# spirlness/qt-raytracer

Hardware: AMD Instinct MI355X
Metric: Msamples/s (rays×bounces/s) at 1920×1080, 8 bounces; 1/2/4/8-GPU scaling (higher is better)
Workload: dtype f32

## Files before the change

### include/hippt.h

```cpp
#ifndef HIPPT_H
#define HIPPT_H

#include <stdbool.h>
#include <stdint.h>

#ifdef __cplusplus
extern "C" {
#endif

bool cudaPathTracerInit(int width, int height, const char **errorMessage);
bool cudaPathTracerRender(int frameIndex, int maxDepth, const unsigned int **hostPixels,
                          const char **errorMessage);
void cudaPathTracerShutdown(void);

bool hipPathTracerInit(int width, int height, const char **errorMessage);
bool hipPathTracerRender(int frameIndex, int maxDepth, const unsigned int **hostPixels,
                         const char **errorMessage);
void hipPathTracerShutdown(void);

typedef struct hipptCamera {
    float origin[3], llc[3], horizontal[3], vertical[3], u[3], v[3];
    float lens_radius;
    float reserved;
} hipptCamera;
// ... 113 lines not shown
    , HIPPT_OPT_LDS_TOP_NODES = 20
    , HIPPT_OPT_BVH_COLLAPSE = 21
    , HIPPT_OPT_BVH_NODE_COST = 22
    , HIPPT_OPT_BVH_LEAF4 = 23
    , HIPPT_OPT_RNG_TABLE = 24
    , HIPPT_OPT_PIXEL_FORMAT = 25
    , HIPPT_OPT_CAMERA_POOL = 26
    , HIPPT_OPT_FUSE_COMBINE = 27
    , HIPPT_OPT_ITEM_ORDER = 28
    , HIPPT_OPT_WAVEFRONT_SORT = 29
    , HIPPT_OPT_CHAIN = 30
    , HIPPT_OPT_CHAIN_AUDIT = 31
    , HIPPT_OPT_PIXEL_TILE = 32
    , HIPPT_OPT_QUERY_SLICE = 33
    , HIPPT_OPT_RENDER_PAD = 34
};
int hipptChainAudit(unsigned int *words, int maxWords);
enum { HIPPT_PIXEL_ARGB = 0, HIPPT_PIXEL_RGBA8 = 1 };
enum { HIPPT_INFO_LDS_TOP_BYTES = 100, HIPPT_INFO_BLOCKS_PER_CU = 101, HIPPT_INFO_CHUNK = 102,
       HIPPT_INFO_CHAIN_CAP = 103,
       HIPPT_INFO_UPDATE_DROPPED = 104 ,
       HIPPT_INFO_RENDER_PAD = 105 };
bool hipptSetOption(int key, long long value);
long long hipptGetOption(int key);
int hipptActiveBvhWidth(void);

const char *hipptLastError(void);

typedef struct hipptBvh hipptBvh;
hipptBvh *hipptBvhBuild(const float *verts, int numTris, float extentHint, const char **errorMessage);
int hipptBvhNodeCount(const hipptBvh *bvh);
int hipptBvhDepth(const hipptBvh *bvh);
void hipptBvhCopy(const hipptBvh *bvh, uint32_t *nodes, int *triOrder);
void hipptBvhFree(hipptBvh *bvh);
bool hipptBvhRefit(hipptBvh *bvh, const float *verts, int numTris, float extentHint, const char **errorMessage);
int hipptBvh4NodeCount(const hipptBvh *bvh);
int hipptBvh4Depth(const hipptBvh *bvh);
// ... 10 lines not shown
```

### qt-raytracer_amd/csrc/hippt_api.cpp

```cpp
#include "../../include/hippt.h"
#include "item_order.h"

#include <hip/hip_runtime.h>

#include <algorithm>
#include <atomic>
#include <cmath>
#include <condition_variable>
#include <cstdio>
#include <cstring>
#include <exception>
#include <memory>
#include <mutex>
#include <stdexcept>
#include <string>
#include <system_error>
#include <thread>
#include <utility>
#include <vector>

#include "bvh_builder.h"
#include "mesh_io.h"
#include "hippt_device.h"
#include "hippt_query.h"
#include "hippt_refit.h"
#include "hippt_slab.h"
#include "hippt_wavefront.h"

struct hipptBvh {
    hippt::Bvh bvh;
    hippt::Bvh4 bvh4;
    std::vector<uint32_t> bvh4q;
};

namespace {

using hippt::CameraF;

using hippt::kStatSlots;
using hippt::kStatWords;
// ... 210 lines not shown
    int leafExit = -1;
    int nodeExit = -1;
    int bvhWidth = 0;
    int stackCap = 0;
    int bvhQuant = -1;
    int ldsTopNodes = -1;
    bool rngTable = false;
    int pixelFormat = HIPPT_PIXEL_ARGB;
    int cameraPool = -1;
    int fuseCombine = -1;
    int itemOrder = -1;
    int pixelTile = -1;
    int chainBatches = -1;
    bool chainAudit = false;
    int renderPad = hippt::slab::kRenderPadDefault;
    long long querySlice = 0;
    std::vector<unsigned> auditWords;
    std::vector<std::pair<int, uint32_t *>> rngTables;
    struct SpareBuf {
        int device;
        void *ptr;
        size_t bytes;
    };
    std::vector<SpareBuf> spare;
    struct Update {
        float *stage[2] = {nullptr, nullptr};
        size_t floats = 0;
        int next = 0;
        std::vector<std::pair<int, hipEvent_t>> busy[2];
        bool hostStale = false;
        int staleBuf = 0;
        hipEvent_t staleEv = nullptr;
    } upd;
    unsigned activeTopBytes = 0;
    int activeBlocksPerCu = 0;
    int activeChunk = 0;
    int activeChainCap = 0;
    int activeRenderPad = 0;
    int activeWidth = 0;
    int blocksPerCu = 0;
    bool ldsScene = true;
    int pathMode = 0;
    unsigned wfSlots = 1u << 27;
    int wfSort = -1;
    hippt::BvhParams bvh;
    double traceMs = 0, combineMs = 0;
    int traceLaunches = 0, combineLaunches = 0;
};

State &S() {
    static State s;
    return s;
// ... 430 lines not shown
        !up(c.mats, s.scene.mats) || !up(c.nodes4, s.scene.nodes4) || !up(c.nodes4q, s.scene.nodes4q))
        return false;
    HIP_TRY(hipMalloc(&c.padDev, 16));
    HIP_TRY(hipMemcpy(c.padDev, &s.scene.pad, sizeof(float), hipMemcpyHostToDevice));
    c.sceneVersion = s.scene.version;
    return true;
}

constexpr float kRenderPadMinSine = 0.3f;
bool render_pad_holds(const SceneHost &sc, bool hostStale, const CameraF &cam) {
    const float M = hostStale ? sc.padSeed : std::max(sc.padSeed, sc.pad * 65536.0f);
    float o = 0.0f;
    for (int k = 0; k < 3; ++k) o = std::max(o, std::fabs(cam.origin[k]));
    const float reach = o + 1.5f * std::fabs(cam.lens_radius);
    return std::isfinite(reach) && reach <= M && sc.minEdgeSine >= kRenderPadMinSine;
}

unsigned packed_ref_bits(int numNodes, int numPrims) {
    const unsigned long long maxMag =
        std::max<unsigned long long>((unsigned long long)std::max(numNodes, 1) * 128ull,
                                     ((unsigned long long)numPrims << 4) + 16ull);
    unsigned bits = 1;
    while ((1ull << (bits - 1)) < maxMag) ++bits;
    return std::max(bits, 8u);
}

constexpr size_t kOrderTables = 4;

int cost_threads() { return int(std::max(1u, std::min(16u, std::thread::hardware_concurrency()))); }

// ... 529 lines not shown
    return true;
}

bool chain_same(const hippt::MeshParams &a, const hippt::MeshParams &b) {
    return a.nodes == b.nodes && a.tris == b.tris && a.shade == b.shade && a.mats == b.mats && a.stats == b.stats &&
           same_cam(a.cam, b.cam) && a.invW == b.invW && a.invH == b.invH && a.width == b.width &&
           a.height == b.height && a.y0 == b.y0 && a.bandRows == b.bandRows && a.rowStride == b.rowStride &&
           a.frames == b.frames && a.maxDepth == b.maxDepth && a.bandPixels == b.bandPixels &&
           a.totalItems == b.totalItems && a.stackDepth == b.stackDepth && a.numNodes == b.numNodes &&
           a.numTris == b.numTris && a.numMats == b.numMats && a.ldsScene == b.ldsScene && a.full == b.full &&
           a.waveThreshold == b.waveThreshold && a.chunk == b.chunk && a.leafExit == b.leafExit &&
           a.nodeExit == b.nodeExit && a.wide == b.wide && a.stackCap == b.stackCap && a.spillCap == b.spillCap &&
           a.spill == b.spill && a.topBytes == b.topBytes && a.refBits == b.refBits && a.runOrder == b.runOrder &&
           a.runCount == b.runCount && a.runTileShift == b.runTileShift && a.rngTable == b.rngTable && a.poolOffset == b.poolOffset &&
           a.poolWords == b.poolWords && a.comb.format == b.comb.format && a.padWord == b.padWord &&
           a.trimScale == b.trimScale;
}

bool launch_chained(Ctx &c, hippt::MeshParams &p, const char **err) {
    Ctx::Chain &ch = c.chain;
    p.chainEpoch = ch.epoch++;
    ch.lastOwn = p.chainSeq;
    ch.pendN = 0;
    if (!c.chainStartEv) HIP_TRY(hipEventCreateWithFlags(&c.chainStartEv, hipEventDisableTiming));
    if (!c.chainEndEv) HIP_TRY(hipEventCreateWithFlags(&c.chainEndEv, hipEventDisableTiming));
    EventPair ev;
    if (!next_events(c, ev, err)) return false;
    HIP_TRY(hipEventRecord(c.chainStartEv, c.stream));
    HIP_TRY(hipEventRecord(ev.a, c.stream));
    HIP_TRY(hippt::launch_mesh(p, int(ch.blocks), false, c.stream));
    HIP_TRY(hipEventRecord(ev.b, c.stream));
// ... 317 lines not shown
                        const bool lambertMega = s.pathMode == 0 && !s.scene.full;
                        p.leafExit = unsigned(s.leafExit >= 0 ? s.leafExit
                                              : ldsScene          ? (lambertMega ? 12 : 4)
                                              : fullMega          ? 12
                                              : lambertGlobal     ? 22
                                                                  : 17);
                        p.nodeExit = unsigned(s.nodeExit >= 0 ? s.nodeExit
                                              : ldsScene  ? 8
                                              : fullMega  ? 16
                                              : lambertGlobal ? 56
                                                              : 48);
                        p.wide = fmt;
                        p.stackCap = stackCap;
                        p.topBytes = topBytes;
                        p.refBits = ldsScene && wide ? packed_ref_bits(numNodes, numTris) : 0u;
                        const bool trims = s.pathMode == 0 && ldsScene && fmt == hippt::kWideFloat && s.renderPad != 0 &&
                                           render_pad_holds(s.scene, s.upd.hostStale, cam);
                        p.padWord = c.padDev;
                        p.trimScale = trims ? hippt::slab::trim_scale(s.renderPad) : 0.0f;
                        s.activeRenderPad = trims ? s.renderPad : 0;
                        p.rngTable = nullptr;
                        p.poolWords = poolWords;
                        if (s.pathMode == 0 && s.itemOrder != 0) {
                            const unsigned *table = nullptr;
                            const int tile = s.pixelTile >= 0 ? s.pixelTile : c.stride == 1 ? 8 : 0;
                            const unsigned tileShift = tile == 8 ? 3u : tile == 16 ? 4u : tile == 32 ? 5u : 6u;
                            if (!ensure_order(c, cam, nf, maxDepth, s.itemOrder == 1, tileShift, &table, err))
                                return false;
                            if (table) {
                                p.runOrder = table;
                                p.runCount = unsigned(c.runCosts.size());
                                p.runTileShift = c.orderKey.tileShift;
                            }
                        }
                        p.poolOffset = unsigned(hippt::mesh_lds_bytes(stackDepth, ldsScene ? numNodes : 0,
// ... 1197 lines not shown
        if (value != 0 && value != 1) return false;
        s.chainAudit = value == 1;
        return true;
    case HIPPT_OPT_PIXEL_TILE:
        if (value != -1 && value != 0 && value != 8 && value != 16 && value != 32) return false;
        s.pixelTile = int(value);
        return true;
    case HIPPT_OPT_QUERY_SLICE:
        if (value < 0 || value > (1LL << 28)) return false;
        s.querySlice = value;
        return true;
    case HIPPT_OPT_RENDER_PAD:
        if (value != 0 && (value < hippt::slab::kRenderPadMin || value > hippt::slab::kRenderPadMax)) return false;
        s.renderPad = int(value);
        return true;
    default: return false;
    }
} catch (const std::exception &e) {
    return false;
} catch (...) {
    return false;
}

extern "C" int hipptActiveBvhWidth(void) try {
    std::lock_guard<std::mutex> g(S().mu);
    return S().activeWidth;
} catch (const std::exception &e) {
    return 0;
} catch (...) {
    return 0;
// ... 24 lines not shown
    case HIPPT_OPT_LDS_TOP_NODES: return s.ldsTopNodes;
    case HIPPT_OPT_BVH_COLLAPSE: return s.bvh.collapse;
    case HIPPT_OPT_BVH_NODE_COST: return (long long)std::lround(s.bvh.nodeCost * 100.0f);
    case HIPPT_OPT_BVH_LEAF4: return s.bvh.maxLeaf4;
    case HIPPT_OPT_RNG_TABLE: return s.rngTable ? 1 : 0;
    case HIPPT_OPT_PIXEL_FORMAT: return s.pixelFormat;
    case HIPPT_OPT_CAMERA_POOL: return s.cameraPool;
    case HIPPT_OPT_FUSE_COMBINE: return s.fuseCombine;
    case HIPPT_OPT_ITEM_ORDER: return s.itemOrder;
    case HIPPT_OPT_WAVEFRONT_SORT: return s.wfSort;
    case HIPPT_OPT_CHAIN: return s.chainBatches;
    case HIPPT_OPT_CHAIN_AUDIT: return s.chainAudit ? 1 : 0;
    case HIPPT_OPT_PIXEL_TILE: return s.pixelTile;
    case HIPPT_OPT_QUERY_SLICE: return s.querySlice;
    case HIPPT_OPT_RENDER_PAD: return s.renderPad;
    case HIPPT_INFO_LDS_TOP_BYTES: return s.activeTopBytes;
    case HIPPT_INFO_BLOCKS_PER_CU: return s.activeBlocksPerCu;
    case HIPPT_INFO_CHUNK: return s.activeChunk;
    case HIPPT_INFO_CHAIN_CAP: return s.activeChainCap;
    case HIPPT_INFO_RENDER_PAD: return s.activeRenderPad;
    case HIPPT_INFO_UPDATE_DROPPED:
        for (Ctx &c : s.ctxs) {
            if (!c.rfUpdated) continue;
            unsigned w[2] = {0, 0};
            if (hipSetDevice(c.device) != hipSuccess || hipStreamSynchronize(c.stream) != hipSuccess ||
                hipMemcpy(w, c.rfWords, sizeof(w), hipMemcpyDeviceToHost) != hipSuccess) {
                (void)hipGetLastError();
                return -1;
            }
            return w[1];
        }
        return 0;
    default: return -1;
    }
} catch (const std::exception &e) {
// ... 107 lines not shown
```

### qt-raytracer_amd/csrc/hippt_device.h

```cpp
#pragma once

#include <hip/hip_runtime.h>

#include <cstdint>

namespace hippt {

struct CameraF {
    float origin[3], llc[3], horizontal[3], vertical[3], u[3], v[3];
    float lens_radius;
    float reserved;
};

struct Sphere4Params {
    float4 *accum;
    uint32_t *out;
    unsigned long long *stats;
    int width, height, y0, rows, rowStride;
    int firstFrame, frames, maxDepth;
    int format;
    uint32_t *hostOut;
};

enum { kPixelArgb = 0, kPixelRgba8 = 1 };

struct CombineParams {
    float4 *accum;
    uint32_t *out;
    const float *scratch;
    unsigned bandPixels, totalItems;
    int firstFrame, frames;
    int format;
};

struct HostFrame {
    uint32_t *host;
    int width, y0, stride;
};

struct MeshParams {
    const float4 *nodes;
    const float4 *tris;
    const float4 *shade;
    const float4 *mats;
    float *scratch;
    unsigned *queue;
    unsigned long long *stats;
    CameraF cam;
    float invW, invH;
    int width, height, y0, bandRows, rowStride;
    int firstFrame, frames, maxDepth;
    unsigned bandPixels, totalItems;
// ... 18 lines not shown
    const uint32_t *rngTable;
    unsigned poolOffset;
    int poolWords;
    CombineParams comb;
    unsigned *combCtr;
    unsigned *chainCtl;
    const unsigned long long *chainBox;
    unsigned chainSeq, chainEpoch, chainRun;
    unsigned chainSlots, chainShift, chainCap;
    int chainStep;
    unsigned chainPosted;
    unsigned chainGroup;
    unsigned *chainAudit;
    const float *padWord;
    float trimScale;
};

constexpr unsigned kChainSlotsMax = 32, kChainBlockWords = 8 * 32 + 32, kChainMarkerWord = 8 * 32;
constexpr unsigned kChainCtlWord = kChainSlotsMax * kChainBlockWords;
constexpr unsigned kChainBoxWord = kChainCtlWord + 128, kChainCtlWords = kChainBoxWord + 8 * 32;
constexpr unsigned kChainMaxShift = 27;
constexpr unsigned kWaveWords = 22;

struct ChainFlushParams {
    CombineParams comb;
    const float *scratch;
    const unsigned *ctl;
    unsigned epoch, lastSeq, slots, shift;
    int step;
    unsigned *audit;
// ... 39 lines not shown
```

### qt-raytracer_amd/csrc/hippt_kernels.hip

```cpp
#include "hippt_trace.h"

#include <algorithm>

#pragma clang fp contract(off)

namespace hippt {
namespace {
using namespace trace;

__device__ __forceinline__ unsigned q8(float c) {
    return unsigned(sqrtf(fminf(fmaxf(c, 0.0f), 1.0f)) * 255.0f);
}

__device__ __forceinline__ uint32_t pack_pixel(float r, float g, float b, int format) {
    if (format == kPixelRgba8) {
        const auto u8 = [](float c) { return unsigned(rintf(sqrtf(fminf(fmaxf(c, 0.0f), 1.0f)) * 255.0f)); };
        return (255u << 24) | (u8(b) << 16) | (u8(g) << 8) | u8(r);
    }
    return (255u << 24) | (q8(r) << 16) | (q8(g) << 8) | q8(b);
}

struct V3 {
    float x, y, z;
};
// ... 122 lines not shown
#endif

#ifndef HIPPT_NUM_SGPR
#define HIPPT_NUM_SGPR 96
#endif
#define HIPPT_SGPR_ATTR __attribute__((amdgpu_num_sgpr(HIPPT_NUM_SGPR)))

#ifndef HIPPT_REJECT_CAP
#define HIPPT_REJECT_CAP 0
#endif

#ifndef HIPPT_PACKED_KEYS
#define HIPPT_PACKED_KEYS 1
#endif

#ifndef HIPPT_LATE_CAM
#define HIPPT_LATE_CAM 0
#endif
#ifndef HIPPT_WIDE_WAVES_PER_EU
#define HIPPT_WIDE_WAVES_PER_EU 7
#endif
template <int UNROLL, bool HOST = false>
__device__ __forceinline__ void combine_pixel(const CombineParams &P, unsigned p, const HostFrame &H = HostFrame{}) {
    float4 acc = P.accum[p];
#pragma unroll UNROLL
    for (int fl = 0; fl < P.frames; ++fl) {
        const size_t k = size_t(fl) * P.bandPixels + p;
        const int f = P.firstFrame + fl;
        const float ff = float(f), fc = float(f + 1);
        const float3 L = *reinterpret_cast<const float3 *>(P.scratch + 3 * k);
// ... 185 lines not shown
    T.cur = kDone;
    T.sp = 0;
    T.leaf = 0;
    T.bestT = INFINITY;
    T.bestI = -1;
    T.bestO = 0x7fffffff;
    float tr = 1, tg = 1, tb = 1;
    bool need = true, fresh = false;
    constexpr unsigned CAP = FULL ? 0u : unsigned(HIPPT_REJECT_CAP);
    unsigned pend = 0;
    unsigned segs = 0, samples = 0;
    unsigned long long nvis = 0, ntest = 0;
    unsigned pc[kProfSlots] = {0};

    constexpr bool FINISH = POOL && !LDS_SCENE;
#ifdef HIPPT_DEBUG_RATE
    const unsigned long long rtStart = __builtin_amdgcn_s_memrealtime();
    unsigned rtBucket = 0, rtSegs0 = 0, rtSamples0 = 0;
    unsigned long long rtRounds = 0, rtLive = 0;
    auto rt_flush = [&](unsigned nb) {
        const unsigned long long a = wave_sum((unsigned long long)(samples - rtSamples0));
        const unsigned wsegs = CHAIN ? __builtin_amdgcn_readfirstlane(ww->segs) : 0u;
        const unsigned long long b = CHAIN ? (unsigned long long)(wsegs - rtSegs0) : wave_sum((unsigned long long)(segs - rtSegs0));
        rtSamples0 = samples;
        rtSegs0 = CHAIN ? wsegs : segs;
        if (__lane_id() == 0) {
            const unsigned k = ((blockIdx.x * 4u + (threadIdx.x >> 6)) % unsigned(kRateSlots) * unsigned(kRateBuckets) +
                                min(rtBucket, unsigned(kRateBuckets - 1))) * 5u;
            atomicAdd(&g_rate[k], a);
            atomicAdd(&g_rate[k + 1], b);
            atomicAdd(&g_rate[k + 2], rtRounds);
            atomicAdd(&g_rate[k + 3], rtLive);
            atomicAdd(&g_rate[k + 4], 1ull);
        }
        rtRounds = rtLive = 0;
        rtBucket = nb;
    };
#endif
    unsigned waveThr = unsigned(P.waveThreshold);
    bool combLeft = CHAIN ? int(__builtin_amdgcn_readfirstlane(cw->c1)) >= int(__builtin_amdgcn_readfirstlane(cw->c0))
                          : P.comb.bandPixels != 0;
    auto comb_step = [&]() { return CHAIN ? combine_chunk_chain(cw) : combine_chunk(P); };
    if (combLeft && (blockIdx.x & 1u) == 0 && threadIdx.x < 64u)
        while (combLeft) combLeft = comb_step();
    for (;;) {
        prof<STATS>(pc, 0);
#ifdef HIPPT_DEBUG_TIMELINE
        if (tlDrained) ++tlRounds;
#endif
#ifdef HIPPT_DEBUG_RATE
        {
            const unsigned nb = unsigned((__builtin_amdgcn_s_memrealtime() - rtStart) / 1000ull);
            if (nb != rtBucket) rt_flush(nb);
            ++rtRounds;
            rtLive += __popcll(__ballot(item != kNone));
        }
#endif
        if (POOL) {
            const unsigned long long m = __ballot(need);
            if (m) {
                const unsigned n = unsigned(__popcll(m));
                const unsigned rank = __builtin_amdgcn_mbcnt_hi(unsigned(m >> 32), __builtin_amdgcn_mbcnt_lo(unsigned(m), 0u));
                const unsigned avail = 64u - poolNext;
                const bool took = need;
                if (need && rank < avail) {
                    need = false;
                    pool_take<POOL>(P, pool, poolNext + rank, item, r, rng);
                }
                if (n > avail) {
                    unsigned it;
                    Ray c{};
                    uint32_t crng = 0;
                    if constexpr (CHAIN) {
                        WorkQueue Q = load_queue(&ww->Q);
                        unsigned raw = kNone, tItem = 0;
                        bool want = true;
                        for (;;) {
                            const unsigned t = __builtin_amdgcn_readfirstlane(cw->t);
                            const bool grp = t == __builtin_amdgcn_readfirstlane(cw->stat);
                            const unsigned nb = grp ? late_field(chainGroup) : 1u;
                            const unsigned got =
                                queue_fetch(want, Q, chain_block(late_field(chainCtl), t, late_field(chainSlots)),
                                            late_field(totalItems) * nb, late_field(chunk), grp, drained, t);
                            if (want && got != kNone) {
                                chain::group_item(got, t, nb, raw, tItem);
                                want = false;
                            }
                            if (!__ballot(want) || !chain_next(Q, cw, view)) break;
                        }
                        store_queue(&ww->Q, Q);
                        it = order_item_late(raw);
                        if (it != kNone) {
                            const int step = int(__builtin_amdgcn_readfirstlane(unsigned(cw->step)));
                            const unsigned fAdd = chain::frame_add(tItem, late_field(chainSeq), step);
                            camera_sample(cam_args_late(), it, c, crng, fAdd);
                            if (unsigned *const audit = late_field(chainAudit))
                                audit_trace(audit, tItem, it, unsigned(late_field(firstFrame)) + fAdd,
                                            late_field(chainEpoch));
                            it |= (tItem & (late_field(chainSlots) - 1u)) << late_field(chainShift);
                        }
                    } else {
                        it = HIPPT_LATE_CAM ? order_item_late(queue_fetch(true, Q, P.queue, P.totalItems, P.chunk, true, drained))
                                            : order_item(P, queue_fetch(true, Q, P.queue, P.totalItems, P.chunk, true, drained));
                        if (it != kNone) {
                            if (HIPPT_LATE_CAM)
                                camera_sample(cam_args_late(), it, c, crng);
                            else
                                camera_sample(P, it, c, crng);
                        }
                    }
#ifdef HIPPT_DEBUG_TIMELINE
                    if (!tlDrained && __ballot(it == kNone)) tlDrained = __builtin_amdgcn_s_memrealtime();
                    tlItems += __popcll(__ballot(it != kNone));
#endif
                    if (it != kNone) prof<STATS>(pc, 1);
                    const unsigned k = __lane_id();
                    pool[k] = __uint_as_float(it);
                    pool[64 + k] = __uint_as_float(crng);
                    pool[128 + k] = c.dx;
                    pool[192 + k] = c.dy;
                    pool[256 + k] = c.dz;
                    if (P.poolWords == kPoolWordsFull) {
                        pool[320 + k] = c.ox;
                        pool[384 + k] = c.oy;
                        pool[448 + k] = c.oz;
                    }
                    poolNext = n - avail;
                    if (need) {
                        need = false;
                        pool_take<POOL>(P, pool, rank - avail, item, r, rng);
                    }
                } else {
                    poolNext += n;
                }
                if (took && item != kNone) {
                    tr = tg = tb = 1.0f;
                    depth = 0;
                    fresh = true;
                }
                if (FINISH && __ballot(took && item == kNone)) waveThr = 0u;
            }
        } else if (__ballot(need)) {
            const unsigned it = HIPPT_LATE_CAM ? order_item_late(queue_fetch(need, Q, P.queue, P.totalItems, P.chunk))
                                               : order_item(P, queue_fetch(need, Q, P.queue, P.totalItems, P.chunk));
#ifdef HIPPT_DEBUG_TIMELINE
            if (!tlDrained && __ballot(need && it == kNone)) tlDrained = __builtin_amdgcn_s_memrealtime();
            tlItems += __popcll(__ballot(it != kNone));
#endif
            if (need) {
                need = false;
                item = it;
                if (it != kNone) {
                    prof<STATS>(pc, 1);
                    if (HIPPT_LATE_CAM)
                        camera_sample(cam_args_late(), it, r, rng);
                    else
                        camera_sample(P, it, r, rng);
                    tr = tg = tb = 1.0f;
                    depth = 0;
                    fresh = true;
                }
            }
        }
        if (fresh) {
            fresh = false;
            prepare(r);
            begin(T);
        }
        if (!__any(busy(T) || pend != 0u)) break;

        if (!CAP || __any(busy(T))) do {
            prof<STATS>(pc, 2);
            if (WIDE)
                traverse_round_wide<nodeF4, STATS, FULL, QUANT, SPILL, LDS_SCENE, TOP, HYBRID, PACKED, HALF,
                                    LDS_SCENE && !FULL>(
                    T, r, my, nodes, tris, nvis, ntest, pc, P.leafExit, P.nodeExit, S, P.topBytes, P.refBits);
            else
                traverse_round<nodeF4, STATS, FULL>(T, r, my, nodes, tris, nvis, ntest, pc, P.leafExit, P.nodeExit);
        } while (__popcll(__ballot(busy(T))) > (FINISH ? waveThr : unsigned(P.waveThreshold)));

        if constexpr (CHAIN) {
            const unsigned long long sm = __ballot(item != kNone && !busy(T) && !(CAP && pend != 0u));
            if (__lane_id() == 0 && sm) atomicAdd(&ww->segs, unsigned(__popcll(sm)));
// ... 217 lines not shown
}

hipError_t launch_mesh(const MeshParams &p, int blocks, bool countTraversal, hipStream_t s) {
    if (p.stackDepth < 1 || p.stackDepth > kStackDepth) return hipErrorInvalidValue;
    if (p.wide && (p.stackCap < 1 || p.stackCap + 2 > p.stackDepth)) return hipErrorInvalidValue;
    const bool lds = p.ldsScene != 0;
    if (p.wide < kWide2 || p.wide > kWideHalf || (lds && p.wide >= kWideQuant)) return hipErrorInvalidValue;
    if (p.topBytes && (lds || p.wide == kWide2 || p.topBytes % (p.wide == kWideQuant ? 64u : 128u) ||
                       p.topBytes > (unsigned(p.numNodes) << (p.wide == kWideQuant ? 6 : 7))))
        return hipErrorInvalidValue;
    if (p.wide == kWideHybrid && !p.topBytes) return hipErrorInvalidValue;
    if (lds && p.wide == kWideFloat && (p.refBits < 8 || p.refBits > 20)) return hipErrorInvalidValue;
    const bool pool = p.poolWords != 0;
    if (pool && ((p.wide != kWideFloat && p.wide != kWideHalf) || (p.poolWords != kPoolWordsPinhole && p.poolWords != kPoolWordsFull)))
        return hipErrorInvalidValue;
    const bool chain = p.chainCtl != nullptr;
    if (chain && (!p.chainBox || p.chainSlots < 2 || p.chainSlots > kChainSlotsMax || (p.chainSlots & (p.chainSlots - 1)) ||
                  p.chainShift > kChainMaxShift || p.totalItems > (1u << p.chainShift) || p.chainCap < 1 ||
                  p.chainCap >= p.chainSlots || p.chainPosted < p.chainSeq || p.chainPosted - p.chainSeq >= p.chainCap ||
                  p.chainGroup < 1 || p.chainGroup > p.chainCap || p.chainPosted - p.chainSeq + 1 < p.chainGroup ||
                  (p.chainGroup > 1 && p.totalItems % 64u) ||
                  p.comb.bandPixels != p.bandPixels || p.comb.frames != p.frames))
        return hipErrorInvalidValue;
    const size_t bytes = mesh_lds_bytes(p.stackDepth, lds ? p.numNodes : 0, lds ? p.numTris : 0, p.wide != 0, p.topBytes,
                                        lds ? p.numMats : 0, p.poolWords);
    if (pool && p.poolOffset != bytes - (size_t(p.poolWords) * 64 + kWaveWords) * (kMeshBlock / 64) * sizeof(float))
        return hipErrorInvalidValue;
    const MeshFn fn = mesh_fn(countTraversal, lds, p.full != 0, p.wide, p.spill != nullptr, pool, chain);
    if (!fn) return hipErrorInvalidValue;
    if (p.wide && (lds || p.topBytes || pool)) {
// ... 40 lines not shown
```

### qt-raytracer_amd/csrc/hippt_trace.h

```cpp
#pragma once

#include "bvh_builder.h"
#include "hippt_chain_logic.h"
#include "hippt_device.h"
#include "hippt_slab.h"

#pragma clang fp contract(off)

namespace hippt {
namespace trace {

constexpr unsigned kNone = 0xffffffffu;
constexpr int kDone = int(0x80000000);

__device__ __forceinline__ uint32_t hash32(uint32_t x) {
    x ^= x >> 16;
    x *= 0x7feb352du;
    x ^= x >> 15;
    x *= 0x846ca68bu;
    x ^= x >> 16;
    return x;
}

__device__ __forceinline__ float rand01(uint32_t &s) {
// ... 476 lines not shown
                                              unsigned epoch, int firstFrame, int step) {
    if (__lane_id() != 0 || n == 0u) return;
    for (int b = c0; b <= c1; ++b) {
        unsigned *const r = audit_record(audit, unsigned(b));
        const unsigned f0 = unsigned(firstFrame + b * step);
        atomicAdd(r + 1, n);
        atomicAdd(reinterpret_cast<unsigned long long *>(r + 4), hsum);
        atomicMax(r + 10, epoch + 1u);
        atomicMax(r + 11, ~epoch);
        atomicMax(r + 12, f0 + 1u);
        atomicMax(r + 13, ~f0);
    }
}

template <typename PP>
__device__ __forceinline__ void camera_sample(const PP &P, unsigned it, Ray &r, uint32_t &rng, unsigned frameAdd = 0u) {
    unsigned fl, p, yb, x;
    divmod(it, P.bandPixels, P.rcpBandPixels, fl, p);
    divmod(p, unsigned(P.width), P.rcpWidth, yb, x);
    const unsigned y = unsigned(P.y0) + yb * unsigned(P.rowStride);
    rng = pixel_seed(x, y, unsigned(P.width), unsigned(P.firstFrame) + fl + frameAdd);
    const float s = (float(x) + rand01(rng)) * P.invW;
    const float t = (float(y) + rand01(rng)) * P.invH;
    float qx, qy;
    for (unsigned tries = 1;; ++tries) {
        qx = rand_pm1(rng);
        qy = rand_pm1(rng);
        if (fmaf(qx, qx, qy * qy) < 1.0f) break;
        escape_cycle(rng, tries);
    }
    const CameraF &C = P.cam;
    const float rx = C.lens_radius * qx, ry = C.lens_radius * qy;
    const float fx = fmaf(C.v[0], ry, C.u[0] * rx);
    const float fy = fmaf(C.v[1], ry, C.u[1] * rx);
    const float fz = fmaf(C.v[2], ry, C.u[2] * rx);
    r.ox = C.origin[0] + fx;
    r.oy = C.origin[1] + fy;
    r.oz = C.origin[2] + fz;
    r.dx = (fmaf(t, C.vertical[0], fmaf(s, C.horizontal[0], C.llc[0])) - C.origin[0]) - fx;
    r.dy = (fmaf(t, C.vertical[1], fmaf(s, C.horizontal[1], C.llc[1])) - C.origin[1]) - fy;
    r.dz = (fmaf(t, C.vertical[2], fmaf(s, C.horizontal[2], C.llc[2])) - C.origin[2]) - fz;
}

__device__ __forceinline__ void store_radiance(float *scratch, unsigned item, float r, float g, float b) {
    *reinterpret_cast<float3 *>(scratch + 3 * size_t(item)) = make_float3(r, g, b);
}

__device__ __forceinline__ void sky_inv(const Ray &r, float inv, float tr, float tg, float tb, float &L0, float &L1,
                                        float &L2) {
    const float uy = inv * r.dy;
    const float al = 0.5f * (uy + 1.0f);
    const float bl = 1.0f - al;
    L0 = tr * fmaf(al, 0.5f, bl);
    L1 = tg * fmaf(al, 0.7f, bl);
    L2 = tb * fmaf(al, 1.0f, bl);
}
// ... 655 lines not shown
```

### qt-raytracer_amd/hippt/__init__.py

```python
from __future__ import annotations

import ctypes
import os
from typing import Optional, Sequence

import numpy as np

from . import scenes

_HERE = os.path.dirname(os.path.abspath(__file__))
LIB_PATH = os.path.join(os.path.dirname(_HERE), "libhippt.so")

SCENE_SPHERE4 = 0
SCENE_MESH = 1

OPT_COUNT_TRAVERSAL = 1
OPT_WAVE_THRESHOLD = 2
OPT_SCRATCH_MB = 3
OPT_CHUNK = 4
OPT_BLOCKS_PER_CU = 5
OPT_LDS_SCENE = 6
OPT_PATH_MODE = 8
OPT_WAVEFRONT_SLOTS = 9
OPT_BVH_LEAF = 10
# ... 8 lines not shown
OPT_BVH_QUANT = 19
OPT_LDS_TOP_NODES = 20
OPT_BVH_COLLAPSE = 21
OPT_BVH_NODE_COST = 22
OPT_BVH_LEAF4 = 23
OPT_RNG_TABLE = 24
OPT_CAMERA_POOL = 26
OPT_FUSE_COMBINE = 27
OPT_ITEM_ORDER = 28
OPT_WAVEFRONT_SORT = 29
OPT_CHAIN = 30
OPT_CHAIN_AUDIT = 31
OPT_PIXEL_TILE = 32
OPT_QUERY_SLICE = 33
OPT_RENDER_PAD = 34
OPT_PIXEL_FORMAT = 25
PIXEL_ARGB = 0
PIXEL_RGBA8 = 1
INFO_LDS_TOP_BYTES = 100
INFO_BLOCKS_PER_CU = 101
INFO_CHUNK = 102
INFO_CHAIN_CAP = 103
INFO_UPDATE_DROPPED = 104
INFO_RENDER_PAD = 105
RAYS_DEVICE = 1
HIT_SPHERE = 1 << 30
HIT_BACKFACE = -(1 << 31)
HIT_MATERIAL_MASK = (1 << 30) - 1
VERTS_DEVICE = 1
SCENE_NODES2 = 0
SCENE_NODES4 = 1
SCENE_PRIMS = 2
SCENE_SHADE = 3

EXPORTS = (
    "cudaPathTracerInit", "cudaPathTracerRender", "cudaPathTracerShutdown",
    "hipPathTracerInit", "hipPathTracerRender", "hipPathTracerShutdown",
    "hipptBuildCamera", "hipptUseBuiltinScene", "hipptUploadMesh", "hipptUploadScene", "hipptReadMesh",
    "hipptFreeMesh", "hipptSetCamera",
# ... 630 lines not shown
```

Baseline: 59370.

## Skip BVH traversal for camera rays provably outside projected scene bounds

On the host, the scene's root bounding box is projected through a pinhole camera to get a conservative screen rectangle, with error bounds. In the persistent pool kernel, when every lane of a wave fetches a pixel outside that rectangle, the wave writes the sky colour directly and skips traversal, the pool round-trip and the lens sampling. It adds a new option, default on, plus per-frame host work and a possible scene settle. Correctness depends on the conservative projection and only applies to pinhole cameras.

```diff
diff --git a/include/hippt.h b/include/hippt.h
--- a/include/hippt.h
+++ b/include/hippt.h
@@ -151,13 +151,15 @@
     , HIPPT_OPT_PIXEL_TILE = 32
     , HIPPT_OPT_QUERY_SLICE = 33
     , HIPPT_OPT_RENDER_PAD = 34
+    , HIPPT_OPT_SKY_RECT = 35
 };
 int hipptChainAudit(unsigned int *words, int maxWords);
 enum { HIPPT_PIXEL_ARGB = 0, HIPPT_PIXEL_RGBA8 = 1 };
 enum { HIPPT_INFO_LDS_TOP_BYTES = 100, HIPPT_INFO_BLOCKS_PER_CU = 101, HIPPT_INFO_CHUNK = 102,
        HIPPT_INFO_CHAIN_CAP = 103,
        HIPPT_INFO_UPDATE_DROPPED = 104 ,
-       HIPPT_INFO_RENDER_PAD = 105 };
+       HIPPT_INFO_RENDER_PAD = 105,
+       HIPPT_INFO_SKY_RECT_PIXELS = 106 };
 bool hipptSetOption(int key, long long value);
 long long hipptGetOption(int key);
 int hipptActiveBvhWidth(void);
diff --git a/qt-raytracer_amd/csrc/hippt_api.cpp b/qt-raytracer_amd/csrc/hippt_api.cpp
--- a/qt-raytracer_amd/csrc/hippt_api.cpp
+++ b/qt-raytracer_amd/csrc/hippt_api.cpp
@@ -24,6 +24,7 @@
 #include "hippt_device.h"
 #include "hippt_query.h"
 #include "hippt_refit.h"
+#include "hippt_sky_rect.h"
 #include "hippt_slab.h"
 #include "hippt_wavefront.h"
 
@@ -264,6 +265,7 @@
     int chainBatches = -1;
     bool chainAudit = false;
     int renderPad = hippt::slab::kRenderPadDefault;
+    bool skyRect = true;
     long long querySlice = 0;
     std::vector<unsigned> auditWords;
     std::vector<std::pair<int, uint32_t *>> rngTables;
@@ -286,6 +288,7 @@
     int activeBlocksPerCu = 0;
     int activeChunk = 0;
     int activeChainCap = 0;
+    long long activeSkyPixels = 0;
     int activeRenderPad = 0;
     int activeWidth = 0;
     int blocksPerCu = 0;
@@ -746,6 +749,23 @@
     for (int k = 0; k < 3; ++k) o = std::max(o, std::fabs(cam.origin[k]));
     const float reach = o + 1.5f * std::fabs(cam.lens_radius);
     return std::isfinite(reach) && reach <= M && sc.minEdgeSine >= kRenderPadMinSine;
+}
+
+hippt::skyrect::Rect sky_rect_of(const SceneHost &sc, const CameraF &cam, int width, int height) {
+    const hippt::skyrect::Rect all = hippt::skyrect::whole(width, height);
+    if (sc.bvh2.nodes.size() < size_t(hippt::kNodeWords)) return all;
+    float lo[3] = {INFINITY, INFINITY, INFINITY}, hi[3] = {-INFINITY, -INFINITY, -INFINITY};
+    bool any = false;
+    for (int slot = 0; slot < 2; ++slot) {
+        if (int32_t(sc.bvh2.nodes[size_t(hippt::node_code_word(2, slot))]) == hippt::leaf_code(0, 0)) continue;
+        any = true;
+        for (int a = 0; a < 3; ++a) {
+            lo[a] = std::min(lo[a], as_float(int(sc.bvh2.nodes[size_t(hippt::node_lo_word(2, slot, a))])));
+            hi[a] = std::max(hi[a], as_float(int(sc.bvh2.nodes[size_t(hippt::node_hi_word(2, slot, a))])));
+        }
+    }
+    if (!any) return all;
+    return hippt::skyrect::sky_rect(cam, width, height, lo, hi, sc.pad, sc.numTris);
 }
 
 unsigned packed_ref_bits(int numNodes, int numPrims) {
@@ -1305,7 +1325,8 @@
            a.spill == b.spill && a.topBytes == b.topBytes && a.refBits == b.refBits && a.runOrder == b.runOrder &&
            a.runCount == b.runCount && a.runTileShift == b.runTileShift && a.rngTable == b.rngTable && a.poolOffset == b.poolOffset &&
            a.poolWords == b.poolWords && a.comb.format == b.comb.format && a.padWord == b.padWord &&
-           a.trimScale == b.trimScale;
+           a.trimScale == b.trimScale && a.skyRect.x0 == b.skyRect.x0 && a.skyRect.y0 == b.skyRect.y0 &&
+           a.skyRect.x1 == b.skyRect.x1 && a.skyRect.y1 == b.skyRect.y1;
 }
 
 bool launch_chained(Ctx &c, hippt::MeshParams &p, const char **err) {
@@ -1653,11 +1674,19 @@
                         p.stackCap = stackCap;
                         p.topBytes = topBytes;
                         p.refBits = ldsScene && wide ? packed_ref_bits(numNodes, numTris) : 0u;
+                        const bool skyWanted = s.pathMode == 0 && poolWords != 0 && s.skyRect &&
+                                               !(s.scene.full && ldsScene && spills && !chained && !cnt);
+                        if (skyWanted && ldsScene && s.upd.hostStale && !s.upd.staleEv) settle_scene();
                         const bool trims = s.pathMode == 0 && ldsScene && fmt == hippt::kWideFloat && s.renderPad != 0 &&
                                            render_pad_holds(s.scene, s.upd.hostStale, cam);
                         p.padWord = c.padDev;
                         p.trimScale = trims ? hippt::slab::trim_scale(s.renderPad) : 0.0f;
                         s.activeRenderPad = trims ? s.renderPad : 0;
+                        const bool skyOn = skyWanted && !s.upd.hostStale;
+                        const hippt::skyrect::Rect sr = skyOn ? sky_rect_of(s.scene, cam, s.width, s.height)
+                                                              : hippt::skyrect::whole(s.width, s.height);
+                        p.skyRect = hippt::SkyRect{sr.x0, sr.y0, sr.x1, sr.y1};
+                        s.activeSkyPixels = hippt::skyrect::pixels_outside(sr, s.width, s.height);
                         p.rngTable = nullptr;
                         p.poolWords = poolWords;
                         if (s.pathMode == 0 && s.itemOrder != 0) {
@@ -2885,6 +2914,10 @@
         if (value != 0 && (value < hippt::slab::kRenderPadMin || value > hippt::slab::kRenderPadMax)) return false;
         s.renderPad = int(value);
         return true;
+    case HIPPT_OPT_SKY_RECT:
+        if (value != 0 && value != 1) return false;
+        s.skyRect = value == 1;
+        return true;
     default: return false;
     }
 } catch (const std::exception &e) {
@@ -2939,11 +2972,13 @@
     case HIPPT_OPT_PIXEL_TILE: return s.pixelTile;
     case HIPPT_OPT_QUERY_SLICE: return s.querySlice;
     case HIPPT_OPT_RENDER_PAD: return s.renderPad;
+    case HIPPT_OPT_SKY_RECT: return s.skyRect ? 1 : 0;
     case HIPPT_INFO_LDS_TOP_BYTES: return s.activeTopBytes;
     case HIPPT_INFO_BLOCKS_PER_CU: return s.activeBlocksPerCu;
     case HIPPT_INFO_CHUNK: return s.activeChunk;
     case HIPPT_INFO_CHAIN_CAP: return s.activeChainCap;
     case HIPPT_INFO_RENDER_PAD: return s.activeRenderPad;
+    case HIPPT_INFO_SKY_RECT_PIXELS: return s.activeSkyPixels;
     case HIPPT_INFO_UPDATE_DROPPED:
         for (Ctx &c : s.ctxs) {
             if (!c.rfUpdated) continue;
diff --git a/qt-raytracer_amd/csrc/hippt_device.h b/qt-raytracer_amd/csrc/hippt_device.h
--- a/qt-raytracer_amd/csrc/hippt_device.h
+++ b/qt-raytracer_amd/csrc/hippt_device.h
@@ -36,6 +36,10 @@
 struct HostFrame {
     uint32_t *host;
     int width, y0, stride;
+};
+
+struct SkyRect {
+    int x0, y0, x1, y1;
 };
 
 struct MeshParams {
@@ -84,6 +88,7 @@
     unsigned *chainAudit;
     const float *padWord;
     float trimScale;
+    SkyRect skyRect;
 };
 
 constexpr unsigned kChainSlotsMax = 32, kChainBlockWords = 8 * 32 + 32, kChainMarkerWord = 8 * 32;
diff --git a/qt-raytracer_amd/csrc/hippt_kernels.hip b/qt-raytracer_amd/csrc/hippt_kernels.hip
--- a/qt-raytracer_amd/csrc/hippt_kernels.hip
+++ b/qt-raytracer_amd/csrc/hippt_kernels.hip
@@ -160,6 +160,11 @@
 #define HIPPT_PACKED_KEYS 1
 #endif
 
+#ifndef HIPPT_SKY_RUNS
+#define HIPPT_SKY_RUNS 1
+#endif
+constexpr unsigned kSkyRunsPerTrip = HIPPT_SKY_RUNS;
+
 #ifndef HIPPT_LATE_CAM
 #define HIPPT_LATE_CAM 0
 #endif
@@ -375,6 +380,7 @@
     unsigned pc[kProfSlots] = {0};
 
     constexpr bool FINISH = POOL && !LDS_SCENE;
+    constexpr bool SKY = POOL && !(FULL && LDS_SCENE && SPILL && !CHAIN && !STATS);
 #ifdef HIPPT_DEBUG_RATE
     const unsigned long long rtStart = __builtin_amdgcn_s_memrealtime();
     unsigned rtBucket = 0, rtSegs0 = 0, rtSamples0 = 0;
@@ -399,6 +405,7 @@
     };
 #endif
     unsigned waveThr = unsigned(P.waveThreshold);
+    unsigned skyRuns = 0;
     bool combLeft = CHAIN ? int(__builtin_amdgcn_readfirstlane(cw->c1)) >= int(__builtin_amdgcn_readfirstlane(cw->c0))
                           : P.comb.bandPixels != 0;
     auto comb_step = [&]() { return CHAIN ? combine_chunk_chain(cw) : combine_chunk(P); };
@@ -417,6 +424,7 @@
             rtLive += __popcll(__ballot(item != kNone));
         }
 #endif
+        bool skyHeld = false;
         if (POOL) {
             const unsigned long long m = __ballot(need);
             if (m) {
@@ -432,6 +440,8 @@
                     unsigned it;
                     Ray c{};
                     uint32_t crng = 0;
+                    float cs = 0.0f, ct = 0.0f;
+                    bool skyLane = false;
                     if constexpr (CHAIN) {
                         WorkQueue Q = load_queue(&ww->Q);
                         unsigned raw = kNone, tItem = 0;
@@ -454,7 +464,9 @@
                         if (it != kNone) {
                             const int step = int(__builtin_amdgcn_readfirstlane(unsigned(cw->step)));
                             const unsigned fAdd = chain::frame_add(tItem, late_field(chainSeq), step);
-                            camera_sample(cam_args_late(), it, c, crng, fAdd);
+                            unsigned px, py;
+                            camera_pixel(cam_args_late(), it, crng, fAdd, px, py, cs, ct);
+                            if (SKY) skyLane = sky_certain(px, py);
                             if (unsigned *const audit = late_field(chainAudit))
                                 audit_trace(audit, tItem, it, unsigned(late_field(firstFrame)) + fAdd,
                                             late_field(chainEpoch));
@@ -464,10 +476,12 @@
                         it = HIPPT_LATE_CAM ? order_item_late(queue_fetch(true, Q, P.queue, P.totalItems, P.chunk, true, drained))
                                             : order_item(P, queue_fetch(true, Q, P.queue, P.totalItems, P.chunk, true, drained));
                         if (it != kNone) {
+                            unsigned px, py;
                             if (HIPPT_LATE_CAM)
-                                camera_sample(cam_args_late(), it, c, crng);
+                                camera_pixel(cam_args_late(), it, crng, 0u, px, py, cs, ct);
                             else
-                                camera_sample(P, it, c, crng);
+                                camera_pixel(P, it, crng, 0u, px, py, cs, ct);
+                            if (SKY) skyLane = sky_certain(px, py);
                         }
                     }
 #ifdef HIPPT_DEBUG_TIMELINE
@@ -475,21 +489,48 @@
                     tlItems += __popcll(__ballot(it != kNone));
 #endif
                     if (it != kNone) prof<STATS>(pc, 1);
-                    const unsigned k = __lane_id();
-                    pool[k] = __uint_as_float(it);
-                    pool[64 + k] = __uint_as_float(crng);
-                    pool[128 + k] = c.dx;
-                    pool[192 + k] = c.dy;
-                    pool[256 + k] = c.dz;
-                    if (P.poolWords == kPoolWordsFull) {
-                        pool[320 + k] = c.ox;
-                        pool[384 + k] = c.oy;
-                        pool[448 + k] = c.oz;
-                    }
-                    poolNext = n - avail;
-                    if (need) {
-                        need = false;
-                        pool_take<POOL>(P, pool, rank - avail, item, r, rng);
+                    if (SKY && __ballot(skyLane) == ~0ull) {
+                        if (CHAIN || HIPPT_LATE_CAM)
+                            camera_dir_pinhole(late_field(cam), cs, ct, c);
+                        else
+                            camera_dir_pinhole(P.cam, cs, ct, c);
+                        float Lr, Lg, Lb;
+                        if (!FULL)
+                            sky_inv(c, rsqrt_rn(fdot(c.dx, c.dy, c.dz, c.dx, c.dy, c.dz)), 1.0f, 1.0f, 1.0f, Lr, Lg, Lb);
+                        else
+                            sky(c, 1.0f, 1.0f, 1.0f, Lr, Lg, Lb);
+                        store_radiance(P.scratch, it, Lr, Lg, Lb);
+                        if constexpr (CHAIN) {
+                            if (__lane_id() == 0) atomicAdd(&ww->segs, 64u);
+                        } else {
+                            ++segs;
+                            ++samples;
+                        }
+                        skyHeld = true;
+                        poolNext = 64;
+                    } else {
+                        if (it != kNone) {
+                            if (CHAIN || HIPPT_LATE_CAM)
+                                camera_ray(late_field(cam), cs, ct, c, crng);
+                            else
+                                camera_ray(P.cam, cs, ct, c, crng);
+                        }
+                        const unsigned k = __lane_id();
+                        pool[k] = __uint_as_float(it);
+                        pool[64 + k] = __uint_as_float(crng);
+                        pool[128 + k] = c.dx;
+                        pool[192 + k] = c.dy;
+                        pool[256 + k] = c.dz;
+                        if (P.poolWords == kPoolWordsFull) {
+                            pool[320 + k] = c.ox;
+                            pool[384 + k] = c.oy;
+                            pool[448 + k] = c.oz;
+                        }
+                        poolNext = n - avail;
+                        if (need) {
+                            need = false;
+                            pool_take<POOL>(P, pool, rank - avail, item, r, rng);
+                        }
                     }
                 } else {
                     poolNext += n;
@@ -499,7 +540,7 @@
                     depth = 0;
                     fresh = true;
                 }
-                if (FINISH && __ballot(took && item == kNone)) waveThr = 0u;
+                if (FINISH && __ballot(took && !need && item == kNone)) waveThr = 0u;
             }
         } else if (__ballot(need)) {
             const unsigned it = HIPPT_LATE_CAM ? order_item_late(queue_fetch(need, Q, P.queue, P.totalItems, P.chunk))
@@ -528,6 +569,8 @@
             prepare(r);
             begin(T);
         }
+        if (SKY && skyHeld && (++skyRuns < kSkyRunsPerTrip || !__any(busy(T) || pend != 0u))) continue;
+        skyRuns = 0;
         if (!__any(busy(T) || pend != 0u)) break;
 
         if (!CAP || __any(busy(T))) do {
@@ -775,6 +818,8 @@
     const bool pool = p.poolWords != 0;
     if (pool && ((p.wide != kWideFloat && p.wide != kWideHalf) || (p.poolWords != kPoolWordsPinhole && p.poolWords != kPoolWordsFull)))
         return hipErrorInvalidValue;
+    if (p.skyRect.x0 < 0 || p.skyRect.y0 < 0 || p.skyRect.x1 < p.skyRect.x0 || p.skyRect.y1 < p.skyRect.y0)
+        return hipErrorInvalidValue;
     const bool chain = p.chainCtl != nullptr;
     if (chain && (!p.chainBox || p.chainSlots < 2 || p.chainSlots > kChainSlotsMax || (p.chainSlots & (p.chainSlots - 1)) ||
                   p.chainShift > kChainMaxShift || p.totalItems > (1u << p.chainShift) || p.chainCap < 1 ||
diff --git a/qt-raytracer_amd/csrc/hippt_sky_rect.h b/qt-raytracer_amd/csrc/hippt_sky_rect.h
--- /dev/null
+++ b/qt-raytracer_amd/csrc/hippt_sky_rect.h
@@ -0,0 +1,104 @@
+#pragma once
+
+#include <cmath>
+
+namespace hippt {
+namespace skyrect {
+
+struct Rect {
+    int x0, y0, x1, y1;
+};
+inline Rect whole(int width, int height) { return Rect{0, 0, width, height}; }
+inline bool is_whole(const Rect &r, int width, int height) {
+    return r.x0 <= 0 && r.y0 <= 0 && r.x1 >= width && r.y1 >= height;
+}
+inline long long pixels_outside(const Rect &r, int width, int height) {
+    const long long w = r.x1 > r.x0 ? r.x1 - r.x0 : 0, h = r.y1 > r.y0 ? r.y1 - r.y0 : 0;
+    return (long long)width * height - w * h;
+}
+
+constexpr double kMaxDirectionErrorPixels = 0.25;
+inline void direction_error_pixels(const double inv[3][3], const double e[3], double sMax, double tMax, double invW,
+                                   double invH, double &px, double &py) {
+    double m[3];
+    for (int r = 0; r < 3; ++r) m[r] = std::fabs(inv[r][0]) * e[0] + std::fabs(inv[r][1]) * e[1] + std::fabs(inv[r][2]) * e[2];
+    if (!(m[0] < 0.5)) {
+        px = py = INFINITY;
+        return;
+    }
+    px = (m[1] + sMax * m[0]) / (1.0 - m[0]) / invW;
+    py = (m[2] + tMax * m[0]) / (1.0 - m[0]) / invH;
+}
+
+template <typename Cam>
+inline Rect sky_rect(const Cam &cam, int width, int height, const float lo[3], const float hi[3], float pad,
+                     int numPrims) {
+    const Rect all = whole(width, height);
+    if (width <= 0 || height <= 0 || numPrims <= 0) return all;
+    if (!(cam.lens_radius == 0.0f)) return all;
+    if (!(pad >= 0.0f) || !std::isfinite(pad)) return all;
+    double o[3], a[3], h[3], v[3], blo[3], bhi[3];
+    for (int k = 0; k < 3; ++k) {
+        o[k] = cam.origin[k];
+        a[k] = double(cam.llc[k]) - o[k];
+        h[k] = cam.horizontal[k];
+        v[k] = cam.vertical[k];
+        blo[k] = double(lo[k]) - double(pad);
+        bhi[k] = double(hi[k]) + double(pad);
+        if (!std::isfinite(o[k]) || !std::isfinite(a[k]) || !std::isfinite(h[k]) || !std::isfinite(v[k]) ||
+            !std::isfinite(blo[k]) || !std::isfinite(bhi[k]) || !(blo[k] <= bhi[k]) || !std::isfinite(cam.u[k]) ||
+            !std::isfinite(cam.v[k]))
+            return all;
+    }
+    auto det3 = [](const double *p, const double *q, const double *r) {
+        return p[0] * (q[1] * r[2] - q[2] * r[1]) - p[1] * (q[0] * r[2] - q[2] * r[0]) +
+               p[2] * (q[0] * r[1] - q[1] * r[0]);
+    };
+    const double det = det3(a, h, v);
+    if (!std::isfinite(det) || det == 0.0) return all;
+    const double invW = double(1.0f / float(width > 1 ? width - 1 : 1));
+    const double invH = double(1.0f / float(height > 1 ? height - 1 : 1));
+    {
+        const double *col[3] = {a, h, v};
+        double inv[3][3], e[3];
+        for (int r = 0; r < 3; ++r) {
+            const double *p = col[(r + 1) % 3], *q = col[(r + 2) % 3];
+            inv[r][0] = (p[1] * q[2] - p[2] * q[1]) / det;
+            inv[r][1] = (p[2] * q[0] - p[0] * q[2]) / det;
+            inv[r][2] = (p[0] * q[1] - p[1] * q[0]) / det;
+        }
+        const double sLim = 1.0 + 2.0 * invW, tLim = 1.0 + 2.0 * invH;
+        for (int k = 0; k < 3; ++k) {
+            const double hv = sLim * std::fabs(h[k]) + tLim * std::fabs(v[k]);
+            e[k] = (2.0 * (std::fabs(double(cam.llc[k])) + hv) + std::fabs(a[k]) + hv) * (1.001 / 16777216.0);
+        }
+        double epx, epy;
+        direction_error_pixels(inv, e, sLim, tLim, invW, invH, epx, epy);
+        if (!(epx <= kMaxDirectionErrorPixels) || !(epy <= kMaxDirectionErrorPixels)) return all;
+    }
+    double sMin = INFINITY, sMax = -INFINITY, tMin = INFINITY, tMax = -INFINITY;
+    for (int c = 0; c < 8; ++c) {
+        double q[3];
+        for (int k = 0; k < 3; ++k) q[k] = (((c >> k) & 1) ? bhi[k] : blo[k]) - o[k];
+        const double l = det3(q, h, v) / det, ls = det3(a, q, v) / det, lt = det3(a, h, q) / det;
+        if (!std::isfinite(l) || !(l > 0.0)) return all;
+        const double px = ls / l / invW, py = lt / l / invH;
+        if (!std::isfinite(px) || !std::isfinite(py)) return all;
+        sMin = std::fmin(sMin, px);
+        sMax = std::fmax(sMax, px);
+        tMin = std::fmin(tMin, py);
+        tMax = std::fmax(tMax, py);
+    }
+    const double ex = 1.0 + double(width) * (1.0 / 1048576.0), ey = 1.0 + double(height) * (1.0 / 1048576.0);
+    auto clampi = [](double d, int hiLim) { return d <= 0.0 ? 0 : d >= double(hiLim) ? hiLim : int(d); };
+    Rect r;
+    r.x0 = clampi(std::ceil(sMin - ex - 1.0), width);
+    r.y0 = clampi(std::ceil(tMin - ey - 1.0), height);
+    r.x1 = clampi(std::floor(sMax + ex) + 1.0, width);
+    r.y1 = clampi(std::floor(tMax + ey) + 1.0, height);
+    if (r.x1 <= r.x0 || r.y1 <= r.y0) return Rect{0, 0, 0, 0};
+    return r;
+}
+
+}
+}
diff --git a/qt-raytracer_amd/csrc/hippt_trace.h b/qt-raytracer_amd/csrc/hippt_trace.h
--- a/qt-raytracer_amd/csrc/hippt_trace.h
+++ b/qt-raytracer_amd/csrc/hippt_trace.h
@@ -514,14 +514,17 @@
 }
 
 template <typename PP>
-__device__ __forceinline__ void camera_sample(const PP &P, unsigned it, Ray &r, uint32_t &rng, unsigned frameAdd = 0u) {
-    unsigned fl, p, yb, x;
+__device__ __forceinline__ void camera_pixel(const PP &P, unsigned it, uint32_t &rng, unsigned frameAdd, unsigned &x,
+                                             unsigned &y, float &s, float &t) {
+    unsigned fl, p, yb;
     divmod(it, P.bandPixels, P.rcpBandPixels, fl, p);
     divmod(p, unsigned(P.width), P.rcpWidth, yb, x);
-    const unsigned y = unsigned(P.y0) + yb * unsigned(P.rowStride);
+    y = unsigned(P.y0) + yb * unsigned(P.rowStride);
     rng = pixel_seed(x, y, unsigned(P.width), unsigned(P.firstFrame) + fl + frameAdd);
-    const float s = (float(x) + rand01(rng)) * P.invW;
-    const float t = (float(y) + rand01(rng)) * P.invH;
+    s = (float(x) + rand01(rng)) * P.invW;
+    t = (float(y) + rand01(rng)) * P.invH;
+}
+__device__ __forceinline__ void camera_ray(const CameraF &C, float s, float t, Ray &r, uint32_t &rng) {
     float qx, qy;
     for (unsigned tries = 1;; ++tries) {
         qx = rand_pm1(rng);
@@ -529,7 +532,6 @@
         if (fmaf(qx, qx, qy * qy) < 1.0f) break;
         escape_cycle(rng, tries);
     }
-    const CameraF &C = P.cam;
     const float rx = C.lens_radius * qx, ry = C.lens_radius * qy;
     const float fx = fmaf(C.v[0], ry, C.u[0] * rx);
     const float fy = fmaf(C.v[1], ry, C.u[1] * rx);
@@ -540,6 +542,23 @@
     r.dx = (fmaf(t, C.vertical[0], fmaf(s, C.horizontal[0], C.llc[0])) - C.origin[0]) - fx;
     r.dy = (fmaf(t, C.vertical[1], fmaf(s, C.horizontal[1], C.llc[1])) - C.origin[1]) - fy;
     r.dz = (fmaf(t, C.vertical[2], fmaf(s, C.horizontal[2], C.llc[2])) - C.origin[2]) - fz;
+}
+__device__ __forceinline__ void camera_dir_pinhole(const CameraF &C, float s, float t, Ray &r) {
+    r.dx = fmaf(t, C.vertical[0], fmaf(s, C.horizontal[0], C.llc[0])) - C.origin[0];
+    r.dy = fmaf(t, C.vertical[1], fmaf(s, C.horizontal[1], C.llc[1])) - C.origin[1];
+    r.dz = fmaf(t, C.vertical[2], fmaf(s, C.horizontal[2], C.llc[2])) - C.origin[2];
+}
+template <typename PP>
+__device__ __forceinline__ void camera_sample(const PP &P, unsigned it, Ray &r, uint32_t &rng, unsigned frameAdd = 0u) {
+    unsigned x, y;
+    float s, t;
+    camera_pixel(P, it, rng, frameAdd, x, y, s, t);
+    camera_ray(P.cam, s, t, r, rng);
+}
+
+__device__ __forceinline__ bool sky_certain(unsigned x, unsigned y) {
+    const SkyRect R = late_field(skyRect);
+    return x - unsigned(R.x0) >= unsigned(R.x1 - R.x0) || y - unsigned(R.y0) >= unsigned(R.y1 - R.y0);
 }
 
 __device__ __forceinline__ void store_radiance(float *scratch, unsigned item, float r, float g, float b) {
diff --git a/qt-raytracer_amd/hippt/__init__.py b/qt-raytracer_amd/hippt/__init__.py
--- a/qt-raytracer_amd/hippt/__init__.py
+++ b/qt-raytracer_amd/hippt/__init__.py
@@ -46,6 +46,7 @@
 OPT_PIXEL_TILE = 32
 OPT_QUERY_SLICE = 33
 OPT_RENDER_PAD = 34
+OPT_SKY_RECT = 35
 OPT_PIXEL_FORMAT = 25
 PIXEL_ARGB = 0
 PIXEL_RGBA8 = 1
@@ -55,6 +56,7 @@
 INFO_CHAIN_CAP = 103
 INFO_UPDATE_DROPPED = 104
 INFO_RENDER_PAD = 105
+INFO_SKY_RECT_PIXELS = 106
 RAYS_DEVICE = 1
 HIT_SPHERE = 1 << 30
 HIT_BACKFACE = -(1 << 31)
```

Result: faster. 61230 (median of 6 runs) (+3.1%).
